# facebookresearch/habitat-lab

Hardware: AMD Instinct MI355X
Metric: env-steps/sec (SPS) PointNav RGB-D 256x256, 64 envs x 128 rollout (higher is better)
Workload: dtype f32; 1 GPU; PointNav SimpleCNN+GRU, 64 envs x 128 steps, 256x256 RGB-D synthetic; envs_per_gpu=64, rollout_steps=128, ppo_epoch=4, num_mini_batch=4, parallelism=dp1

## Files before the change

habitat-lab_amd/csrc/engine.hip:

```cpp
#include <string.h>

#include <algorithm>

#include <string>
#include <vector>

#include "engine.h"

using namespace hab;

static void plan_tm_workspace(hab_policy* e, Arena& wk);
void add_tail_params(hab_policy* e) {
    const hab_policy_desc& d = e->d;
    const int H = d.hidden;
    const std::string rn = "net.state_encoder.rnn.";
    for (int l = 0; l < d.rnn_layers; ++l) {
        const int in = l == 0 ? e->rnn_in : H;
        const std::string sfx = "_l" + std::to_string(l);
        e->i_wih.push_back(add_param(e, rn + "weight_ih" + sfx, {e->G_ * H, in}));
        e->i_whh.push_back(add_param(e, rn + "weight_hh" + sfx, {e->G_ * H, H}));
        e->i_bih.push_back(add_param(e, rn + "bias_ih" + sfx, {e->G_ * H}));
        e->i_bhh.push_back(add_param(e, rn + "bias_hh" + sfx, {e->G_ * H}));
    }
    if (d.action_dist == HAB_DIST_GAUSSIAN) {
// ... 434 lines not shown
        HAB_TRY(rnn_frag_init(hidden0 + (size_t)l * H, rows, hidden_env_stride, masks, rows, frag_env, frag_start, F, H,
                              e->WK + e->w_hinit + (size_t)l * F * H, s, env_first_frame));
        if (e->d.rnn_type == HAB_RNN_LSTM)
            HAB_TRY(rnn_frag_init(hidden0 + (size_t)(L + l) * H, rows, hidden_env_stride, masks, rows, frag_env, frag_start, F, H,
                                  e->WK + e->w_cinit + (size_t)l * F * H, s, env_first_frame));
    }
    return HAB_OK;
}
static int rnn_tm_forward(hab_policy* e, const hab_obs* obs, const int* rows, const float* hidden0, int hidden_env_stride,
                          const uint8_t* masks, int B, int n, hipStream_t stream) {
    float* W = e->WK;
    const int H = e->d.hidden, L = e->L, NC = e->form.chunks, T = B / n, Tc = (T + NC - 1) / NC;
    HAB_TRY(tm_setup(e, 2 * NC + 4));
    hipStream_t sB = e->s2;
    uint8_t* fmask = reinterpret_cast<uint8_t*>(W + e->w_fmask);
    HAB_TRY(rnn_tm_prepare(masks, rows, B, fmask, reinterpret_cast<int*>(W + e->w_iota), stream));
    HAB_TRY(rnn_state_init(e, hidden0, hidden_env_stride, rows, masks, nullptr, nullptr, n, nullptr, stream));
    for (int c = 0; c < NC; ++c) {
        const int t0 = c * Tc, t1 = std::min(T, t0 + Tc);
        if (t0 >= t1) break;
        HAB_TRY(encoder_forward(e, obs, masks, rows, B, stream, t0 * n, (t1 - t0) * n));
        HAB_TRY(tm_order(e, c, stream, sB));
        for (int l = 0; l < L; ++l) {
            Probe pr(e, HAB_PROBE_RNN_FWD, sB);
            HAB_TRY(rnn_tm_layer_forward(e->d.rnn_type, H, layer_params(e, l), layer_work(e, l), layer_x(e, l), layer_ld(e, l),
                                         W + e->w_hinit + (size_t)l * n * H, W + e->w_cinit + (size_t)l * n * H, fmask, n, T, t0, t1,
                                         W + e->w_ws2, e->ws2_floats, sB));
        }
    }
    return tm_order(e, NC, sB, stream);
}
static int rnn_packed_forward(hab_policy* e, const int* rows, const float* hidden0, int hidden_env_stride, const uint8_t* masks,
                              const hab_pack_info* pack, int n, hipStream_t stream) {
    float* W = e->WK;
    const int H = e->d.hidden, L = e->L;
    const PackInfo pk = pack_info(pack, n);
    HAB_TRY(rnn_state_init(e, hidden0, hidden_env_stride, rows, masks, pk.frag_env, pk.frag_start, pk.F, pack->env_first_frame, stream));
    if (e->form.wave) {
        RnnLayerParams lps[4]; RnnWork wks[4]; const float* hin[4]; const float* cin[4];
        for (int l = 0; l < L; ++l) {
            lps[l] = layer_params(e, l); wks[l] = layer_work(e, l);
            hin[l] = W + e->w_hinit + (size_t)l * pk.F * H; cin[l] = W + e->w_cinit + (size_t)l * pk.F * H;
        }
        Probe pr(e, HAB_PROBE_RNN_FWD, stream);
        const int rc = rnn_seq_wave_forward(e->d.rnn_type, H, L, lps, wks, layer_x(e, 0), layer_ld(e, 0), hin, cin, pk, W + e->w_ws,
                                            e->ws_floats, stream);
        return rc == 1 ? HAB_ERR_UNSUPPORTED : rc;
    }
    for (int l = 0; l < L; ++l) {
        Probe pr(e, HAB_PROBE_RNN_FWD, stream);
        HAB_TRY(rnn_seq_layer_forward(e->d.rnn_type, H, layer_params(e, l), layer_work(e, l), layer_x(e, l), layer_ld(e, l),
                                      W + e->w_hinit + (size_t)l * pk.F * H, W + e->w_cinit + (size_t)l * pk.F * H, pk, W + e->w_ws,
                                      e->ws_floats, stream));
    }
    return HAB_OK;
}

extern "C" int hab_policy_evaluate(hab_policy* e, const hab_obs* obs, const int* rows, const float* hidden0,
                                   int hidden_env_stride, const uint8_t* masks, const int64_t* actions,
                                   const hab_pack_info* pack, int B, int n, float* value, float* log_prob, float* entropy,
                                   hipStream_t stream) {
    if (!e || !e->P || !obs || !hidden0 || !masks || !actions || !pack || B <= 0 || n <= 0 || B > e->d.max_frames) return HAB_ERR_ARG;
    if (!pack->env_first_frame && (B % n)) return HAB_ERR_ARG;
    if (pack->P != B || pack->F <= 0 || pack->F > B || pack->max_len <= 0) return HAB_ERR_ARG;
    float* W = e->WK;
    const int H = e->d.hidden, L = e->L;
    e->form = rnn_form(e, rows, pack, B, n);
    if (e->form.chunks > 0) {
        HAB_TRY(rnn_tm_forward(e, obs, rows, hidden0, hidden_env_stride, masks, B, n, stream));
    } else {
        HAB_TRY(encoder_forward(e, obs, masks, rows, B, stream));
        HAB_TRY(rnn_packed_forward(e, rows, hidden0, hidden_env_stride, masks, pack, n, stream));
    }
    const float* feats = W + e->w_out[L - 1];
    if (e->d.action_dist == HAB_DIST_GAUSSIAN) {
        GaussHeadsArgs ga;
        ga.B = B; ga.H = H; ga.A = e->d.num_actions; ga.K = e->head_K; ga.flags = e->d.gauss_flags; ga.mode = 0;
        ga.min_std = e->d.gauss_min_std; ga.max_std = e->d.gauss_max_std;
        ga.feats = feats; ga.feats_ld = H; ga.w = e->p(e->i_aw); ga.b = e->p(e->i_ab);
        ga.std_param = e->i_astd >= 0 ? e->p(e->i_astd) : nullptr; ga.w_critic = e->p(e->i_cw); ga.b_critic = e->p(e->i_cb);
        ga.actions_in = reinterpret_cast<const float*>(actions); ga.rows = rows; ga.noise = nullptr; ga.actions_out = nullptr;
        ga.value = value ? value : W + e->w_value; ga.logp = log_prob ? log_prob : W + e->w_logp;
        ga.entropy = entropy ? entropy : W + e->w_ent; ga.saved = W + e->w_gsaved;
        HAB_TRY(gauss_heads_forward(ga, stream));
    } else {
    HeadsArgs ha;
        ha.B = B; ha.H = H; ha.A = e->d.num_actions; ha.mode = 0;
        ha.feats = feats; ha.feats_ld = H; ha.w_actor = e->p(e->i_aw); ha.b_actor = e->p(e->i_ab); ha.w_critic = e->p(e->i_cw); ha.b_critic = e->p(e->i_cb);
        ha.actions_in = actions; ha.rows = rows; ha.noise = nullptr; ha.actions_out = nullptr;
        ha.value = value ? value : W + e->w_value; ha.logp = log_prob ? log_prob : W + e->w_logp;
        ha.entropy = entropy ? entropy : W + e->w_ent;
        ha.probs = W + e->w_probs; ha.logits_n = W + e->w_logitsn;
        HAB_TRY(heads_forward(ha, stream));
    }
    e->last_B = B;
    e->last_n = pack->env_first_frame ? 0 : n;
    e->last_masks = masks;
    return HAB_OK;
}

extern "C" int hab_policy_final_hidden(hab_policy* e, float* hidden_out, hipStream_t stream) {
    if (!e || !hidden_out || e->last_B <= 0 || e->last_n <= 0) return HAB_ERR_ARG;
    const int H = e->d.hidden, L = e->L, n = e->last_n, B = e->last_B;
    const int Lh = e->d.rnn_type == HAB_RNN_LSTM ? 2 * L : L;
    for (int l = 0; l < L; ++l) {
        HAB_TRY(copy_rows(e->WK + e->w_out[l] + (size_t)(B - n) * H, nullptr, H, hidden_out + (size_t)l * H, Lh * H, n, H, stream));
        if (e->d.rnn_type == HAB_RNN_LSTM)
            HAB_TRY(copy_rows(e->WK + e->w_c[l] + (size_t)(B - n) * H, nullptr, H, hidden_out + (size_t)(L + l) * H, Lh * H, n, H, stream));
    }
    return HAB_OK;
}

__global__ void add_rows_kernel(float* __restrict__ dst, const float* __restrict__ src, long long n) {
    for (long long i = (long long)blockIdx.x * blockDim.x + threadIdx.x; i < n; i += (long long)gridDim.x * blockDim.x) dst[i] += src[i];
}
__global__ void add_masked_cols_kernel(float* __restrict__ dst, int ldd, const float* __restrict__ src, const float* __restrict__ x, int ldx,
                                       int B, int H) {
    const long long n = (long long)B * H;
    for (long long i = (long long)blockIdx.x * blockDim.x + threadIdx.x; i < n; i += (long long)gridDim.x * blockDim.x) {
        const int f = (int)(i / H), c = (int)(i % H);
        if (x[(size_t)f * ldx + c] > 0.f) dst[(size_t)f * ldd + c] += src[i];
    }
}
extern "C" int hab_policy_set_extra_grads(hab_policy* e, const float* d_rnn_output, const float* d_perception_embed) {
    if (!e) return HAB_ERR_ARG;
    if (d_perception_embed && e->Cin == 0) return HAB_ERR_ARG;
    e->xg_feat = d_rnn_output; e->xg_perc = d_perception_embed;
    return HAB_OK;
}

static int cnn_dgrad(hab_policy* e, int64_t f0, int nB, hipStream_t s) {
    float* W = e->WK;
    float* ws = W + e->w_ws;
    const int64_t m1 = (int64_t)e->c1.Ho() * e->c1.Wo() * 32, m2 = (int64_t)e->c2.Ho() * e->c2.Wo() * 64, m3 = e->fc_in;
    ConvDesc c2 = e->c2, c3 = e->c3;
    c2.B = c3.B = nB;
    { Probe pr(e, HAB_PROBE_FC_DGRAD, s);
      HAB_TRY(linear_dgrad(W + e->w_drnnin + f0 * e->rnn_ld, e->rnn_ld, e->PK + e->pk_fc, e->fc_in, nullptr, 0, 0, W + e->w_da3 + f0 * m3,
                           e->fc_in, nB, e->fc_in, e->d.hidden, 0, ws, e->ws_floats, s)); }
    { Probe pr(e, HAB_PROBE_CONV3_DGRAD, s);
      HAB_TRY(conv_dgrad(c3, W + e->w_da3 + f0 * m3, e->PK + e->pk_c3d, W + e->w_a2 + f0 * m2, nullptr, W + e->w_da2 + f0 * m2, ws,
                         e->ws_floats, s)); }
    { Probe pr(e, HAB_PROBE_CONV2_DGRAD, s);
      HAB_TRY(conv_dgrad(c2, W + e->w_da2 + f0 * m2, e->PK + e->pk_c2d, W + e->w_a1 + f0 * m1, nullptr, W + e->w_da1 + f0 * m1, ws,
                         e->ws_floats, s)); }
    return HAB_OK;
}
static int rnn_tm_backward(hab_policy* e, int B, hipStream_t stream) {
    float* W = e->WK;
    const int H = e->d.hidden, L = e->L, n = e->last_n, T = B / n, NC = e->form.chunks, Tc = (T + NC - 1) / NC;
    hipStream_t sB = e->s2;
    const uint8_t* fmask = reinterpret_cast<const uint8_t*>(W + e->w_fmask);
    const int* iota = reinterpret_cast<const int*>(W + e->w_iota);
    HAB_TRY(tm_order(e, NC + 1, stream, sB));
    for (int c = NC - 1; c >= 0; --c) {
        const int t0 = c * Tc, t1 = std::min(T, t0 + Tc);
        if (t0 >= t1) continue;
        for (int l = L - 1; l >= 0; --l) {
            Probe pr(e, HAB_PROBE_RNN_BWD, sB);
            HAB_TRY(rnn_tm_layer_backward(e->d.rnn_type, H, layer_params(e, l), layer_work(e, l), layer_dout(e, l), layer_dx(e, l), layer_ld(e, l),
                                          l == 0 ? layer_x(e, 0) : nullptr, layer_ld(e, l), H, fmask, iota, n, T, t0, t1,
                                          W + e->w_scratch + (size_t)l * 2 * n * H, W + e->w_ws2, e->ws2_floats, sB));
        }
        if (!e->rn) {
            HAB_TRY(tm_order(e, NC + 2 + c, sB, stream));
            HAB_TRY(cnn_dgrad(e, (int64_t)t0 * n, (t1 - t0) * n, stream));
        }
    }
    for (int l = L - 1; l >= 0; --l)
        HAB_TRY(rnn_tm_layer_param_grads(e->d.rnn_type, H, layer_params(e, l), layer_work(e, l), layer_x(e, l), layer_ld(e, l), B, W + e->w_ws2,
                                         e->ws2_floats, sB));
    return HAB_OK;
}
static int rnn_packed_backward(hab_policy* e, const hab_pack_info* pack, hipStream_t stream) {
    float* W = e->WK;
    const int H = e->d.hidden, L = e->L;
    const PackInfo pk = pack_info(pack, e->last_n);
    const bool blind0 = !e->rn && e->Cin == 0, nofc = e->Cin == 0;
    const float* x0 = layer_x(e, 0);
    if (e->form.wave) {
        RnnLayerParams lps[4]; RnnWork wks[4]; const float* wiht[4];
        for (int l = 0; l < L; ++l) { lps[l] = layer_params(e, l); wks[l] = layer_work(e, l); wiht[l] = l ? e->PK + e->pk_wiht[l] : nullptr; }
        Probe pr(e, HAB_PROBE_RNN_BWD, stream);
        const int rc = rnn_seq_wave_backward(e->d.rnn_type, H, L, lps, wiht, wks, x0, e->rnn_ld, layer_dout(e, L - 1), blind0 ? nullptr : layer_dx(e, 0),
                                             e->rnn_ld, nofc ? nullptr : x0, e->rnn_ld, nofc ? 0 : H, pk, W + e->w_scratch, W + e->w_ws, e->ws_floats,
                                             stream);
        return rc == 1 ? HAB_ERR_UNSUPPORTED : rc;
    }
    for (int l = L - 1; l >= 0; --l) {
        Probe pr(e, HAB_PROBE_RNN_BWD, stream);
        HAB_TRY(rnn_seq_layer_backward(e->d.rnn_type, H, layer_params(e, l), layer_work(e, l), layer_x(e, l), layer_ld(e, l), layer_dout(e, l),
                                       (blind0 && l == 0) ? nullptr : layer_dx(e, l), layer_ld(e, l), (l == 0 && !nofc) ? x0 : nullptr,
                                       layer_ld(e, l), nofc ? 0 : H, pk, W + e->w_scratch, W + e->w_ws, e->ws_floats, stream));
    }
    return HAB_OK;
}

static int policy_backward_impl(hab_policy* e, const hab_obs* obs, const int* rows, const int64_t* actions,
                                const hab_pack_info* pack, const float* d_value, const float* d_log_prob,
                                const float* d_entropy, hipStream_t stream) {
    if (!e || !e->P || !e->G || !obs || !actions || !pack || !d_value || !d_log_prob || !d_entropy || e->last_B <= 0)
        return HAB_ERR_ARG;
    e->comm_err = HAB_OK;
    float* W = e->WK;
    float* ws = W + e->w_ws;
    const int H = e->d.hidden, L = e->L, B = e->last_B, A = e->d.num_actions;
    e->cur_stream = stream;
    e->comm_first = -1;
    const float* feats = W + e->w_out[L - 1];
    if (e->d.action_dist == HAB_DIST_GAUSSIAN) {
        const int K = e->head_K;
        GaussHeadsBwdArgs gb;
        gb.B = B; gb.H = H; gb.A = A; gb.K = K; gb.d_value = d_value; gb.d_logp = d_log_prob; gb.d_entropy = d_entropy;
        gb.actions = reinterpret_cast<const float*>(actions); gb.rows = rows; gb.saved = W + e->w_gsaved;
        gb.w = e->p(e->i_aw); gb.w_critic = e->p(e->i_cw); gb.dfeat = W + e->w_dfeat; gb.dz = W + e->w_dzv; gb.dv_out = W + e->w_dv;
        HAB_TRY(gauss_heads_backward(gb, stream));
        HAB_TRY(linear_wgrad(W + e->w_dzv, 8, feats, H, e->g(e->i_aw), H, B, K, H, 0, 0, 0, ws, e->ws_floats, stream));
        HAB_TRY(colsum(W + e->w_dzv, 8, B, K, e->g(e->i_ab), 0, ws, e->ws_floats, stream));
        if (e->i_astd >= 0) HAB_TRY(colsum(W + e->w_dzv + A, 8, B, A, e->g(e->i_astd), 0, ws, e->ws_floats, stream));
        HAB_TRY(linear_wgrad(W + e->w_dv, 1, feats, H, e->g(e->i_cw), H, B, 1, H, 0, 0, 0, ws, e->ws_floats, stream));
        HAB_TRY(colsum(W + e->w_dv, 1, B, 1, e->g(e->i_cb), 0, ws, e->ws_floats, stream));
    } else {
    HeadsBwdArgs hb;
        hb.B = B; hb.H = H; hb.A = A; hb.d_value = d_value; hb.d_logp = d_log_prob; hb.d_entropy = d_entropy;
        hb.actions = actions; hb.rows = rows; hb.probs = W + e->w_probs; hb.logits_n = W + e->w_logitsn;
        hb.w_actor = e->p(e->i_aw); hb.w_critic = e->p(e->i_cw); hb.dfeat = W + e->w_dfeat; hb.dzv = W + e->w_dzv; hb.dv_out = W + e->w_dv;
        HAB_TRY(heads_backward(hb, stream));
        HAB_TRY(linear_wgrad(W + e->w_dzv, 8, feats, H, e->g(e->i_aw), H, B, A, H, 0, 0, 0, ws, e->ws_floats, stream));
        HAB_TRY(linear_wgrad(W + e->w_dv, 1, feats, H, e->g(e->i_cw), H, B, 1, H, 0, 0, 0, ws, e->ws_floats, stream));
        HAB_TRY(colsum(W + e->w_dzv, 8, B, A, e->g(e->i_ab), 0, ws, e->ws_floats, stream));
        HAB_TRY(colsum(W + e->w_dv, 1, B, 1, e->g(e->i_cb), 0, ws, e->ws_floats, stream));
    }
    const int NC = e->form.chunks;
    if (e->xg_feat || e->xg_perc) {
        if (NC > 0) return HAB_ERR_UNSUPPORTED;
        if (e->xg_feat) {
            add_rows_kernel<<<(int)std::min<long long>(1024, cdivl((long long)B * H, 256)), 256, 0, stream>>>(W + e->w_dfeat, e->xg_feat, (long long)B * H);
            HAB_LAUNCH_CHECK();
        }
    }
    if (NC > 0) {
        HAB_TRY(rnn_tm_backward(e, B, stream));
    } else {
        HAB_TRY(rnn_packed_backward(e, pack, stream));
        if (e->xg_perc) {
            add_masked_cols_kernel<<<(int)std::min<long long>(1024, cdivl((long long)B * H, 256)), 256, 0, stream>>>(
                W + e->w_drnnin, e->rnn_ld, e->xg_perc, W + e->w_rnnin, e->rnn_ld, B, H);
            HAB_LAUNCH_CHECK();
        }
        if (!e->rn && e->Cin == 0) {
            grad_tail_ready(e, e->i_wih[0]);
            return HAB_OK;
        }
    }
    if (e->rn) {
        if (NC > 0) HAB_TRY(tm_order(e, 2 * NC + 3, e->s2, stream));
        Probe pr(e, HAB_PROBE_ENC_BWD, stream);
        return resnet_encoder_backward(e, obs, e->last_masks, rows, B, stream);
    }
    const float* dfc = W + e->w_drnnin;
    { Probe pr(e, HAB_PROBE_FC_WGRAD, stream);
      HAB_TRY(linear_wgrad(dfc, e->rnn_ld, W + e->w_a3, e->fc_in, e->g(e->i_fcw), e->fc_in, B, H, e->fc_in, 32, e->fc_in / 32, 0,
                           ws, e->ws_floats, stream)); }
    HAB_TRY(colsum(dfc, e->rnn_ld, B, H, e->g(e->i_fcb), 0, ws, e->ws_floats, stream));
    if (NC > 0) HAB_TRY(tm_order(e, 2 * NC + 3, e->s2, stream));
    grad_tail_ready(e, e->i_fcw);
    if (NC == 0) HAB_TRY(cnn_dgrad(e, 0, B, stream));
    ConvDesc c1 = e->c1, c2 = e->c2, c3 = e->c3;
    c1.B = c2.B = c3.B = B;
    { Probe pr(e, HAB_PROBE_CONV3_WGRAD, stream);
      HAB_TRY(conv_wgrad(c3, W + e->w_a2, W + e->w_da3, e->g(e->i_c3w), e->g(e->i_c3b), ws, e->ws_floats, stream)); }
    { Probe pr(e, HAB_PROBE_CONV2_WGRAD, stream);
      HAB_TRY(conv_wgrad(c2, W + e->w_a1, W + e->w_da2, e->g(e->i_c2w), e->g(e->i_c2b), ws, e->ws_floats, stream)); }
    ObsView ov;
    ov.rgb = e->d.has_rgb ? obs->rgb : nullptr; ov.depth = e->d.has_depth ? obs->depth : nullptr; ov.rows = rows;
    ov.H = e->d.H; ov.W = e->d.W; ov.C = e->Cin;
    { Probe pr(e, HAB_PROBE_CONV1_WGRAD, stream);
      HAB_TRY(obs_conv_wgrad(c1, ov, W + e->w_da1, e->g(e->i_c1w), e->g(e->i_c1b), ws, e->ws_floats, stream)); }
    return HAB_OK;
}
extern "C" int hab_policy_backward(hab_policy* e, const hab_obs* obs, const int* rows, const int64_t* actions,
                                   const hab_pack_info* pack, const float* d_value, const float* d_log_prob,
                                   const float* d_entropy, hipStream_t stream) {
    const int rc = policy_backward_impl(e, obs, rows, actions, pack, d_value, d_log_prob, d_entropy, stream);
    if (e) e->xg_feat = e->xg_perc = nullptr;
    return (rc == HAB_OK && e && e->comm_err != HAB_OK) ? e->comm_err : rc;
}

extern "C" int hab_policy_tap(hab_policy* e, int which, const float** ptr, int64_t* floats) {
    if (!e || !ptr || !floats || e->last_B <= 0) return HAB_ERR_ARG;
    const int64_t B = e->last_B;
    float* W = e->WK;
    if (e->rn && which != HAB_TAP_RNN_IN && which != HAB_TAP_RNN_OUT) return resnet_tap(e, which, ptr, floats);
    if (!e->rn && e->Cin == 0 && (which == HAB_TAP_CONV1 || which == HAB_TAP_CONV2 || which == HAB_TAP_CONV3)) return HAB_ERR_ARG;
    switch (which) {
        case HAB_TAP_CONV1: *ptr = W + e->w_a1; *floats = B * e->c1.Ho() * e->c1.Wo() * 32; break;
        case HAB_TAP_CONV2: *ptr = W + e->w_a2; *floats = B * e->c2.Ho() * e->c2.Wo() * 64; break;
        case HAB_TAP_CONV3: *ptr = W + e->w_a3; *floats = B * e->fc_in; break;
        case HAB_TAP_RNN_IN: *ptr = W + e->w_rnnin; *floats = B * e->rnn_ld; break;
        case HAB_TAP_RNN_OUT: *ptr = W + e->w_out[e->L - 1]; *floats = B * e->d.hidden; break;
        default: return HAB_ERR_ARG;
    }
    return HAB_OK;
}
```

habitat-lab_amd/csrc/gemm_ops.hip:

```cpp
#include "igemm.h"
#include "igemm_dma.h"
#include "igemm_dma_wgrad.h"
#include "igemm_bf3.h"
#include "igemm_bf3_ws.h"
#include "dense_bf3.h"
#include "obs_conv_bf3.h"
#include "obs_conv_bf3_ws.h"
#include "obs_conv_patch.h"
#include "wgrad3x3_bf3.h"
#include "conv2_fwd_strip.h"
#include "conv2_dgrad_strip.h"
#include "obs_wgrad_bf3.h"
#include "conv_patch_bf3.h"
#include "wgrad3x3_patch.h"
#include "prob_build.h"
#include <stdlib.h>

#include <atomic>

#include "../../include/habitat_amd.h"

namespace hab {

static bool no_dma() { static const bool v = hab_env_flag("HAB_NO_DMA"); return v; }
static bool no_merged_dgrad() { static const bool v = hab_env_flag("HAB_NO_MERGED_DGRAD"); return v; }
static bool no_patch() { static const bool v = hab_env_flag("HAB_NO_PATCH"); return v; }
static std::atomic<int> g_bf3_mode{-1};
static int bf3_mode() {
    int m = g_bf3_mode.load(std::memory_order_relaxed);
    if (m < 0) {
        static const int from_env = hab_env_int("HAB_BF3", 2047);
        int expected = -1;
        g_bf3_mode.compare_exchange_strong(expected, from_env, std::memory_order_relaxed);
        m = g_bf3_mode.load(std::memory_order_relaxed);
    }
    return m;
}
int matrix_path_bits() { return bf3_mode(); }
extern "C" int hab_set_matrix_path(int mode) {
    const int prev = bf3_mode();
    if (mode >= 0) g_bf3_mode.store(mode, std::memory_order_relaxed);
    return prev;
}


template <class P, int TM, int TN, int WM, int WN>
static int bf3_launch(const P& p, float* ws, size_t ws_floats, int target_blocks, hipStream_t stream) {
    constexpr bool WS_SHAPE = P::A_RC && P::B_RC && TM == 2 && TN == 2 && WM == 2 && WN == 2;
    if constexpr (WS_SHAPE) {
        constexpr int ws_min_k = 2048;
        if ((bf3_mode() & 32) && p.K >= ws_min_k) return igemm_bf3_ws_launch<P, TM, TN, WM, WN, 4>(p, ws, ws_floats, target_blocks, stream);
    }
    return igemm_bf3_launch<P, TM, TN, WM, WN>(p, ws, ws_floats, target_blocks, stream);
}

template <class P>
static int run_igemm(const P& p, float* ws, size_t ws_floats, hipStream_t stream, int target_blocks = 1024) {
    if (P::A_RC || P::B_RC) target_blocks = 256;
    constexpr bool WG = !P::A_RC && !P::B_RC && AKv<P>::value == 4;
    if constexpr (P::A_RC && P::B_RC) {
        if ((bf3_mode() & 1) && p.M > 64) {
            if (p.N <= 32) return bf3_launch<P, 2, 1, 4, 1>(p, ws, ws_floats, target_blocks, stream);
            if (p.N <= 64) {
                if (p.M >= 256 * 512 && p.K >= 576) return bf3_launch<P, 2, 2, 4, 1>(p, ws, ws_floats, target_blocks, stream);
                return bf3_launch<P, 1, 2, 4, 1>(p, ws, ws_floats, target_blocks, stream);
            }
            return bf3_launch<P, 2, 2, 2, 2>(p, ws, ws_floats, target_blocks, stream);
        }
    } else if constexpr (AKv<P>::value == 4) {
        if ((bf3_mode() & 4) && p.M > 64) {
            if (p.N <= 32) {
                if constexpr (WG) {
                    if (p.M % 96 == 0 || cdiv(p.M, 96) * 96 < cdiv(p.M, 256) * 256)
                        return bf3_launch<P, 1, 1, 3, 1>(p, ws, ws_floats, target_blocks, stream);
                }
                return bf3_launch<P, 2, 1, 4, 1>(p, ws, ws_floats, target_blocks, stream);
            }
            if (p.N <= 64) {
                if constexpr (WG) {
                    if (p.M % 96 == 0 || cdiv(p.M, 96) * 96 < cdiv(p.M, 128) * 128)
                        return bf3_launch<P, 1, 2, 3, 1>(p, ws, ws_floats, target_blocks, stream);
                }
                return bf3_launch<P, 1, 2, 4, 1>(p, ws, ws_floats, target_blocks, stream);
            }
            return bf3_launch<P, 2, 2, 2, 2>(p, ws, ws_floats, target_blocks, stream);
        }
    }
    if constexpr (std::is_same_v<P, ConvFwdProb> || std::is_same_v<P, ConvDgradProb>) {
        if (p.dma_ok() && p.M > 64 && !no_dma()) {
            if (p.N <= 32) return igemm_dma_launch<P, 2, 1, 4, 1, false>(p, ws, ws_floats, target_blocks, stream);
            if (p.N <= 64) return igemm_dma_launch<P, 1, 2, 4, 1, false>(p, ws, ws_floats, target_blocks, stream);
            if (p.N <= 128) return igemm_dma_launch<P, 2, 2, 2, 2, true>(p, ws, ws_floats, target_blocks, stream);
        }
    }
    if (p.N <= 32) {
        if (p.M <= 64) return igemm_launch<P, 1, 1, 2, 1>(p, ws, ws_floats, target_blocks, stream);
        if constexpr (WG) {
            if (p.M % 96 == 0 || cdiv(p.M, 96) * 96 < cdiv(p.M, 256) * 256)
                return igemm_launch<P, 1, 1, 3, 1>(p, ws, ws_floats, target_blocks, stream);
        }
        return igemm_launch<P, 2, 1, 4, 1>(p, ws, ws_floats, target_blocks, stream);
    } else if (p.N <= 64) {
        if (p.M <= 64) return igemm_launch<P, 1, 1, 2, 2>(p, ws, ws_floats, target_blocks, stream);
        if constexpr (WG) {
            if (p.M % 96 == 0 || cdiv(p.M, 96) * 96 < cdiv(p.M, 128) * 128)
                return igemm_launch<P, 1, 2, 3, 1>(p, ws, ws_floats, target_blocks, stream);
        }
        return igemm_launch<P, 1, 2, 4, 1>(p, ws, ws_floats, target_blocks, stream);
    } else {
        if (p.M <= 64) return igemm_launch<P, 1, 2, 2, 2>(p, ws, ws_floats, target_blocks, stream);
        return igemm_launch<P, 2, 2, 2, 2>(p, ws, ws_floats, target_blocks, stream);
    }
}

int conv_fwd(const ConvDesc& d, const float* x, const float* wf, const float* bias, float* y, int relu, float* ws,
             size_t ws_floats, hipStream_t stream) {
    ConvFwdProb p;
    HAB_TRY(build(p, d, x, wf, bias, y, relu));
    if ((bf3_mode() & 256) && (bf3_mode() & 1)) {
        const int rc = conv2_fwd_strip(p, ws, ws_floats, stream);
        if (rc != 1) return rc;
    }
    if ((bf3_mode() & 16) && d.stride == 1 && d.KH == 3 && d.KW == 3 && p.M > 64) {
        PatchGeom gq{};
        gq.in = x; gq.Hi = d.H; gq.Wi = d.W; gq.Ci = d.C; gq.Ho = p.g.Ho; gq.Wo = p.g.Wo; gq.KH = 3; gq.KW = 3;
        gq.off_h = -d.pad; gq.off_w = -d.pad; gq.flip = 0;
        const int rc = conv_patch_bf3_dispatch(p, gq, ws, ws_floats, stream);
        if (rc != 1) return rc;
    }
    return run_igemm(p, ws, ws_floats, stream);
}
int64_t obs_conv_weight_image_floats() { return ((int64_t)OCP_W_ELEMS + 1) / 2 + 4; }
int obs_conv_weight_image(const float* wf, int Cout, int KH, int KW, int C, void* img, hipStream_t stream) {
    return obs_conv_patch_weight_image(wf, Cout, KH, KW, C, reinterpret_cast<unsigned short*>(img), stream);
}
int obs_conv_fwd(const ConvDesc& d, const ObsView& obs, const float* wf, const float* bias, float* y, int relu, float* ws,
                 size_t ws_floats, hipStream_t stream, const void* wimg) {
    ObsConvFwdProb p;
    HAB_TRY(build(p, d, obs, wf, bias, y, relu));
    if ((bf3_mode() & 64) && (bf3_mode() & 2) && p.quad) {
        const int rc = obs_conv_patch_launch(p, ws, ws_floats, stream, reinterpret_cast<const unsigned short*>(wimg));
        if (rc != 1) return rc;
    }
    if ((bf3_mode() & 32) && (bf3_mode() & 2) && p.quad && p.M > 64) {
        const int rc = obs_conv_bf3_ws_launch(p, ws, ws_floats, stream);
        if (rc != 1) return rc;
    }
    if ((bf3_mode() & 2) && p.quad && p.M > 64) {
        const int rc = obs_conv_bf3_launch<2>(p, ws, ws_floats, stream);
        if (rc != 1) return rc;
    }
    return run_igemm(p, ws, ws_floats, stream);
}
__global__ void dgrad_empty_class_kernel(ConvDgradProb p) {
    const long long total = (long long)p.g.B * p.Hc * p.Wc * p.N;
    for (long long e = (long long)blockIdx.x * blockDim.x + threadIdx.x; e < total; e += (long long)gridDim.x * blockDim.x)
        p.store((int)(e / p.N), (int)(e % p.N), 0.f);
}

int conv_dgrad(const ConvDesc& d, const float* dy, const float* wd, const float* mask, const float* add, float* dx,
               float* ws, size_t ws_floats, hipStream_t stream) {
    if ((bf3_mode() & 512) && (bf3_mode() & 1)) {
        const int rc = conv2_dgrad_strip(d, dy, wd, mask, add, dx, stream);
        if (rc != 1) return rc;
    }
    if (d.stride > 1 && !no_dma() && !no_merged_dgrad()) {
        ConvDgradMergedProb q;
        HAB_TRY(check_conv(d));
        q.g = make_geom(d);
        if (ConvDgradMergedProb::applicable(q.g)) {
            q.dy = dy; q.w = wd; q.mask = mask; q.add = add; q.dx = dx;
            q.finish();
            if ((bf3_mode() & 1) && q.M > 64) {
                if (q.N <= 32) return bf3_launch<ConvDgradMergedProb, 2, 1, 4, 1>(q, ws, ws_floats, 256, stream);
                if (q.N <= 64) return bf3_launch<ConvDgradMergedProb, 1, 2, 4, 1>(q, ws, ws_floats, 256, stream);
                return bf3_launch<ConvDgradMergedProb, 2, 2, 2, 2>(q, ws, ws_floats, 256, stream);
            }
            if (q.dma_ok()) {
                if (q.N <= 32) return igemm_dma_launch<ConvDgradMergedProb, 2, 1, 4, 1, false>(q, ws, ws_floats, 1024, stream);
                if (q.N <= 64) return igemm_dma_launch<ConvDgradMergedProb, 1, 2, 4, 1, false>(q, ws, ws_floats, 1024, stream);
                return igemm_dma_launch<ConvDgradMergedProb, 2, 2, 2, 2, false>(q, ws, ws_floats, 1024, stream);
            }
        }
    }
    for (int ph = 0; ph < d.stride; ++ph)
        for (int pw = 0; pw < d.stride; ++pw) {
            ConvDgradProb p;
            HAB_TRY(build(p, d, dy, wd, mask, add, dx, ph, pw));
            if (p.Hc <= 0 || p.Wc <= 0) continue;
            if ((bf3_mode() & 16) && d.stride == 1 && d.KH == 3 && d.KW == 3 && p.M > 64 && p.K > 0) {
                PatchGeom gq{};
                gq.in = dy; gq.Hi = p.g.Ho; gq.Wi = p.g.Wo; gq.Ci = d.Cout; gq.Ho = d.H; gq.Wo = d.W; gq.KH = 3; gq.KW = 3;
                gq.off_h = d.pad - 2; gq.off_w = d.pad - 2; gq.flip = 1;
                const int rc = conv_patch_bf3_dispatch(p, gq, ws, ws_floats, stream);
                if (rc == HAB_OK) continue;
                if (rc != 1) return rc;
            }
            if (p.K <= 0) {
                p.M = d.B * p.Hc * p.Wc;
                dgrad_empty_class_kernel<<<1024, 256, 0, stream>>>(p);
                HAB_LAUNCH_CHECK();
                continue;
            }
            HAB_TRY(run_igemm(p, ws, ws_floats, stream));
        }
    return HAB_OK;
}
int conv_wgrad(const ConvDesc& d, const float* x, const float* dy, float* dw_oihw, float* dbias, float* ws, size_t ws_floats,
               hipStream_t stream) {
    ConvWgradProb p;
    HAB_TRY(build(p, d, x, dy, dw_oihw, dbias));
    if (ws && (bf3_mode() & 8) && (bf3_mode() & 128) && wgrad3x3_bf3_shape(p)) {
        const int rc = wgrad3x3_bf3(p, ws, ws_floats, stream);
        if (rc != 1) return rc;
    }
    if (ws && wgrad3x3_patch_ok(p) && !no_patch() && !(bf3_mode() & 8)) {
        ConvWgradProb q = p;
        q.colsum = nullptr;
        if (dbias) HAB_TRY(colsum(dy, p.N, p.K, p.N, dbias, 0, ws, ws_floats, stream));
        return wgrad3x3_patch(q, ws, ws_floats, stream);
    }
    if (ws && d.pad == 0 && p.N <= 32 && !no_dma() && !(bf3_mode() & 8)) {
        ConvWgradProb q = p;
        q.colsum = nullptr;
        if (wgrad_dma_ok(q)) {
            if (dbias) HAB_TRY(colsum(dy, p.N, p.K, p.N, dbias, 0, ws, ws_floats, stream));
            if ((q.M % 288 == 0) || (cdiv(q.M, 288) * 288 < cdiv(q.M, 256) * 256)) return igemm_dma_wgrad_launch<3, 3, 1>(q, ws, ws_floats, 1024, stream);
            return igemm_dma_wgrad_launch<2, 4, 1>(q, ws, ws_floats, 1024, stream);
        }
    }
    return run_igemm(p, ws, ws_floats, stream);
}
int obs_conv_wgrad(const ConvDesc& d, const ObsView& obs, const float* dy, float* dw_oihw, float* dbias, float* ws,
                   size_t ws_floats, hipStream_t stream) {
    ObsConvWgradProb p;
    HAB_TRY(build(p, d, obs, dy, dw_oihw, dbias));
    if ((bf3_mode() & 2) && p.quad && p.K > 4096) {
        const int rc = obs_wgrad_bf3_launch(p, ws, ws_floats, stream);
        if (rc != 1) return rc;
    }
    return run_igemm(p, ws, ws_floats, stream);
}
static bool dense_on() { return (bf3_mode() & 1024) && (bf3_mode() & 1); }
static bool dense_worth(long long M, long long N, long long K) {
    if (bf3_mode() & 2048) return true;
    static const long long min_flop = (long long)hab_env_int("HAB_DENSE_MIN_MFLOP", 4000) * 1000000LL;
    return 2 * M * N * K >= min_flop;
}
int linear_fwd(const float* x, int ldx, const float* w, int ldw, const float* bias, float* y, int ldy, int M, int N, int K,
               int relu, int accumulate, float* ws, size_t ws_floats, hipStream_t stream) {
    LinearFwdProb p;
    HAB_TRY(build(p, x, ldx, w, ldw, bias, y, ldy, M, N, K, relu, accumulate));
    if (dense_on() && dense_worth(M, N, K)) {
        DenseArgs g{};
        g.M = M; g.N = N; g.K = K; g.a = x; g.lda = ldx; g.b = w; g.ldb = ldw; g.c = y; g.ldc = ldy; g.bias = bias; g.relu = relu;
        g.accumulate = accumulate; g.partial = ws;
        g.a_bytes = ((long long)(M - 1) * ldx + K) * 4; g.b_bytes = ((long long)(N - 1) * ldw + K) * 4;
        if (dense_bf3_ok(g, false, false)) {
            g.nsplit = ws ? dense_bf3_splits(g, ws_floats) : 1;
            HAB_TRY((dense_bf3_launch<0, 0>(g, stream)));
            if (g.nsplit > 1) {
                igemm_splitk_reduce<LinearFwdProb>(p, ws, g.nsplit, stream);
                HAB_LAUNCH_CHECK();
            }
            return HAB_OK;
        }
    }
    return run_igemm(p, ws, ws_floats, stream);
}
int linear_dgrad(const float* dy, int lddy, const float* w, int ldw, const float* mask, int ldmask, int mask_cols, float* dx,
                 int lddx, int M, int Nin, int Kout, int accumulate, float* ws, size_t ws_floats, hipStream_t stream) {
    LinearDgradProb p;
    HAB_TRY(build(p, dy, lddy, w, ldw, mask, ldmask, mask_cols, dx, lddx, M, Nin, Kout, accumulate));
    if (dense_on() && !mask && dense_worth(M, Nin, Kout)) {
        DenseArgs g{};
        g.M = M; g.N = Nin; g.K = Kout; g.a = dy; g.lda = lddy; g.b = w; g.ldb = ldw; g.c = dx; g.ldc = lddx; g.accumulate = accumulate;
        g.partial = ws;
        g.a_bytes = ((long long)(M - 1) * lddy + Kout) * 4; g.b_bytes = ((long long)(Kout - 1) * ldw + Nin) * 4;
        if (dense_bf3_ok(g, false, true)) {
            g.nsplit = ws ? dense_bf3_splits(g, ws_floats) : 1;
            HAB_TRY((dense_bf3_launch<0, 1>(g, stream)));
            if (g.nsplit > 1) {
                igemm_splitk_reduce<LinearDgradProb>(p, ws, g.nsplit, stream);
                HAB_LAUNCH_CHECK();
            }
            return HAB_OK;
        }
    }
    return run_igemm(p, ws, ws_floats, stream);
}
int linear_wgrad(const float* dy, int lddy, const float* x, int ldx, float* dw, int lddw, int Mrows, int Nout, int Kin,
                 int perm_c, int perm_hw, int accumulate, float* ws, size_t ws_floats, hipStream_t stream) {
    LinearWgradProb p;
    HAB_TRY(build(p, dy, lddy, x, ldx, dw, lddw, Mrows, Nout, Kin, perm_c, perm_hw, accumulate));
    if (dense_on() && dense_worth(Nout, Kin, Mrows)) {
        DenseArgs g{};
        g.M = Nout; g.N = Kin; g.K = Mrows; g.a = dy; g.lda = lddy; g.b = x; g.ldb = ldx; g.c = dw; g.ldc = lddw; g.accumulate = accumulate;
        g.perm_c = perm_c; g.perm_hw = perm_hw; g.partial = ws;
        g.a_bytes = ((long long)(Mrows - 1) * lddy + Nout) * 4; g.b_bytes = ((long long)(Mrows - 1) * ldx + Kin) * 4;
        if (dense_bf3_ok(g, true, true)) {
            g.nsplit = ws ? dense_bf3_splits(g, ws_floats) : 1;
            HAB_TRY((dense_bf3_launch<1, 1>(g, stream)));
            if (g.nsplit > 1) {
                igemm_splitk_reduce<LinearWgradProb>(p, ws, g.nsplit, stream);
                HAB_LAUNCH_CHECK();
            }
            return HAB_OK;
        }
    }
    return run_igemm(p, ws, ws_floats, stream);
}

__global__ void __launch_bounds__(256) colsum_stage1(const float* __restrict__ a, int lda, int M, int N, int rows_per_block,
                                                     float* __restrict__ partial) {
    const int cw = N < 64 ? N : 64;
    const int rl = 256 / cw;
    const int c = threadIdx.x % cw, r = threadIdx.x / cw;
    const int n = blockIdx.x * cw + c;
    __shared__ float sm[256];
    const int m_begin = blockIdx.y * rows_per_block, m_end = min(M, m_begin + rows_per_block);
    float s0 = 0.f, s1 = 0.f;
    if (r < rl && n < N) {
        int m = m_begin + r;
        for (; m + rl < m_end; m += 2 * rl) {
            s0 += a[(size_t)m * lda + n];
            s1 += a[(size_t)(m + rl) * lda + n];
        }
        if (m < m_end) s0 += a[(size_t)m * lda + n];
    }
    sm[threadIdx.x] = s0 + s1;
    __syncthreads();
    if (r == 0 && n < N) {
        float t = 0.f;
        for (int q = 0; q < rl; ++q) t += sm[q * cw + c];
        partial[(size_t)blockIdx.y * N + n] = t;
    }
}
__global__ void __launch_bounds__(256) colsum_stage2(const float* __restrict__ partial, int nblocks, int N, float* __restrict__ out,
                                                     int accumulate) {
    __shared__ float sm[4][64];
    const int c = threadIdx.x & 63, r = threadIdx.x >> 6;
    const int n = blockIdx.x * 64 + c;
    float s0 = 0.f, s1 = 0.f, s2 = 0.f, s3 = 0.f;
    if (n < N) {
        int b = r;
        for (; b + 12 < nblocks; b += 16) {
            s0 += partial[(size_t)b * N + n];
            s1 += partial[(size_t)(b + 4) * N + n];
            s2 += partial[(size_t)(b + 8) * N + n];
            s3 += partial[(size_t)(b + 12) * N + n];
        }
        for (; b < nblocks; b += 4) s0 += partial[(size_t)b * N + n];
    }
    const float s = (s0 + s1) + (s2 + s3);
    sm[r][c] = s;
    __syncthreads();
    if (r == 0 && n < N) {
        const float t = (sm[0][c] + sm[1][c]) + (sm[2][c] + sm[3][c]);
        out[n] = accumulate ? out[n] + t : t;
    }
}

int colsum(const float* a, int lda, int M, int N, float* out, int accumulate, float* ws, size_t ws_floats, hipStream_t stream) {
    if (M <= 0 || N <= 0 || !a || !out || !ws) return HAB_ERR_ARG;
    const int cw = N < 64 ? N : 64;
    const int colblocks = cdiv(N, cw);
    int chunks = cdiv(1024, colblocks);
    if (chunks > cdiv(M, 16)) chunks = cdiv(M, 16);
    while (chunks > 1 && (size_t)chunks * N > ws_floats) chunks >>= 1;
    if ((size_t)chunks * N > ws_floats) return HAB_ERR_ARG;
    const int rpb = cdiv(M, chunks);
    chunks = cdiv(M, rpb);
    colsum_stage1<<<dim3(colblocks, chunks), 256, 0, stream>>>(a, lda, M, N, rpb, ws);
    HAB_LAUNCH_CHECK();
    colsum_stage2<<<cdiv(N, 64), 256, 0, stream>>>(ws, chunks, N, out, accumulate);
    HAB_LAUNCH_CHECK();
    return HAB_OK;
}

__global__ void repack_conv_kernel(const float* __restrict__ w, float* __restrict__ wf, float* __restrict__ wd, int Cout,
                                   int Cin, int KH, int KW, int cpad) {
    const int total = Cout * cpad * KH * KW;
    for (int e = blockIdx.x * blockDim.x + threadIdx.x; e < total; e += gridDim.x * blockDim.x) {
        const int ci = e % cpad;
        int t = e / cpad;
        const int kw = t % KW; t /= KW;
        const int kh = t % KH;
        const int co = t / KH;
        const float v = (ci < Cin) ? w[(((size_t)co * Cin + ci) * KH + kh) * KW + kw] : 0.f;
// ... 145 lines not shown
```

Before: 61740 env-steps/s.

## Add patch-based obs conv1 wgrad kernel and start RNN backward earlier

Adds a new MFMA bf16x3 weight-gradient kernel for the 8x8 stride-4 first conv on raw RGB-D observations. It stages row-band patches in an LDS ring so overlapping input rows are reused across output rows, and it is enabled by default through a new mode bit. It also moves the stream-ordering event for the RNN backward stream to right after the heads backward, so RNN backward can overlap the head weight-gradient GEMMs. The new kernel adds more bf16 split arithmetic and a split-K reduction. It only covers a narrow shape set and falls back otherwise.

Measured after the change: 54950 env-steps/s. -11.0%, worse.

```diff
diff --git a/habitat-lab_amd/csrc/engine.hip b/habitat-lab_amd/csrc/engine.hip
--- a/habitat-lab_amd/csrc/engine.hip
+++ b/habitat-lab_amd/csrc/engine.hip
@@ -610,7 +610,6 @@
     hipStream_t sB = e->s2;
     const uint8_t* fmask = reinterpret_cast<const uint8_t*>(W + e->w_fmask);
     const int* iota = reinterpret_cast<const int*>(W + e->w_iota);
-    HAB_TRY(tm_order(e, NC + 1, stream, sB));
     for (int c = NC - 1; c >= 0; --c) {
         const int t0 = c * Tc, t1 = std::min(T, t0 + Tc);
         if (t0 >= t1) continue;
@@ -666,6 +665,7 @@
     e->cur_stream = stream;
     e->comm_first = -1;
     const float* feats = W + e->w_out[L - 1];
+    const int NC = e->form.chunks;
     if (e->d.action_dist == HAB_DIST_GAUSSIAN) {
         const int K = e->head_K;
         GaussHeadsBwdArgs gb;
@@ -673,6 +673,7 @@
         gb.actions = reinterpret_cast<const float*>(actions); gb.rows = rows; gb.saved = W + e->w_gsaved;
         gb.w = e->p(e->i_aw); gb.w_critic = e->p(e->i_cw); gb.dfeat = W + e->w_dfeat; gb.dz = W + e->w_dzv; gb.dv_out = W + e->w_dv;
         HAB_TRY(gauss_heads_backward(gb, stream));
+        if (NC > 0) HAB_TRY(tm_order(e, NC + 1, stream, e->s2));
         HAB_TRY(linear_wgrad(W + e->w_dzv, 8, feats, H, e->g(e->i_aw), H, B, K, H, 0, 0, 0, ws, e->ws_floats, stream));
         HAB_TRY(colsum(W + e->w_dzv, 8, B, K, e->g(e->i_ab), 0, ws, e->ws_floats, stream));
         if (e->i_astd >= 0) HAB_TRY(colsum(W + e->w_dzv + A, 8, B, A, e->g(e->i_astd), 0, ws, e->ws_floats, stream));
@@ -684,12 +685,12 @@
         hb.actions = actions; hb.rows = rows; hb.probs = W + e->w_probs; hb.logits_n = W + e->w_logitsn;
         hb.w_actor = e->p(e->i_aw); hb.w_critic = e->p(e->i_cw); hb.dfeat = W + e->w_dfeat; hb.dzv = W + e->w_dzv; hb.dv_out = W + e->w_dv;
         HAB_TRY(heads_backward(hb, stream));
+        if (NC > 0) HAB_TRY(tm_order(e, NC + 1, stream, e->s2));
         HAB_TRY(linear_wgrad(W + e->w_dzv, 8, feats, H, e->g(e->i_aw), H, B, A, H, 0, 0, 0, ws, e->ws_floats, stream));
         HAB_TRY(linear_wgrad(W + e->w_dv, 1, feats, H, e->g(e->i_cw), H, B, 1, H, 0, 0, 0, ws, e->ws_floats, stream));
         HAB_TRY(colsum(W + e->w_dzv, 8, B, A, e->g(e->i_ab), 0, ws, e->ws_floats, stream));
         HAB_TRY(colsum(W + e->w_dv, 1, B, 1, e->g(e->i_cb), 0, ws, e->ws_floats, stream));
     }
-    const int NC = e->form.chunks;
     if (e->xg_feat || e->xg_perc) {
         if (NC > 0) return HAB_ERR_UNSUPPORTED;
         if (e->xg_feat) {
diff --git a/habitat-lab_amd/csrc/gemm_ops.hip b/habitat-lab_amd/csrc/gemm_ops.hip
--- a/habitat-lab_amd/csrc/gemm_ops.hip
+++ b/habitat-lab_amd/csrc/gemm_ops.hip
@@ -11,6 +11,7 @@
 #include "conv2_fwd_strip.h"
 #include "conv2_dgrad_strip.h"
 #include "obs_wgrad_bf3.h"
+#include "obs_wgrad_patch.h"
 #include "conv_patch_bf3.h"
 #include "wgrad3x3_patch.h"
 #include "prob_build.h"
@@ -29,7 +30,7 @@
 static int bf3_mode() {
     int m = g_bf3_mode.load(std::memory_order_relaxed);
     if (m < 0) {
-        static const int from_env = hab_env_int("HAB_BF3", 2047);
+        static const int from_env = hab_env_int("HAB_BF3", 2047 | 8192);
         int expected = -1;
         g_bf3_mode.compare_exchange_strong(expected, from_env, std::memory_order_relaxed);
         m = g_bf3_mode.load(std::memory_order_relaxed);
@@ -235,6 +236,10 @@
                    size_t ws_floats, hipStream_t stream) {
     ObsConvWgradProb p;
     HAB_TRY(build(p, d, obs, dy, dw_oihw, dbias));
+    if ((bf3_mode() & 2) && (bf3_mode() & 8192) && p.quad && p.K > 1024) {
+        const int rc = obs_wgrad_patch_launch(p, ws, ws_floats, stream);
+        if (rc != 1) return rc;
+    }
     if ((bf3_mode() & 2) && p.quad && p.K > 4096) {
         const int rc = obs_wgrad_bf3_launch(p, ws, ws_floats, stream);
         if (rc != 1) return rc;
diff --git a/habitat-lab_amd/csrc/obs_wgrad_patch.h b/habitat-lab_amd/csrc/obs_wgrad_patch.h
--- /dev/null
+++ b/habitat-lab_amd/csrc/obs_wgrad_patch.h
@@ -0,0 +1,229 @@
+#pragma once
+#include "obs_wgrad_bf3.h"
+
+namespace hab {
+
+constexpr int OWP_P = 72;
+constexpr int OWP_SLOT = 24 * OWP_P + 32;
+constexpr int OWP_RING = 8 * OWP_SLOT;
+constexpr int OWP_BP = 32 * OWP_P;
+constexpr size_t OWP_LDS_BYTES = (size_t)(OWP_RING + 2 * 3 * OWP_BP) * 2;
+static_assert(OWP_LDS_BYTES >= 256 * 32 * 4, "the cross-wave reduction reuses the tile buffers");
+static_assert(OWP_LDS_BYTES % 16 == 0 && (OWP_SLOT * 2) % 16 == 0, "16-byte fragment reads");
+
+struct ObsWgradPatchGeom {
+    FastDiv dHo;
+    int tiles, tiles_per_wg;
+};
+
+__global__ void __launch_bounds__(256, 2) obs_wgrad_patch_kernel(const ObsConvWgradProb p, const ObsWgradPatchGeom gg, float* __restrict__ partial) {
+    extern __shared__ __attribute__((aligned(16))) unsigned short smem16[];
+    unsigned short* T = smem16;
+    unsigned short* B0 = T + OWP_RING;
+    unsigned short* B1 = B0 + 3 * OWP_BP;
+
+    const int t = threadIdx.x;
+    const int lane = t & 63, wave = t >> 6;
+    const int li = lane & 31, hi = lane >> 5;
+    const ConvGeom& g = p.g;
+
+    const int qpr = g.W >> 2;
+    const int a_r = t / qpr, a_x4 = t - a_r * qpr;
+    const bool a_ok = t < g.W;
+    const size_t a_pix = (size_t)(a_ok ? a_r : 0) * g.W + 4 * (a_ok ? a_x4 : 0);
+    const int b_coq = t >> 5, b_kr = t & 31;
+    const bool b_col_ok = b_coq * 4 < p.N;
+
+    const int tile_begin = blockIdx.x * gg.tiles_per_wg;
+    const int tile_end = min(gg.tiles, tile_begin + gg.tiles_per_wg);
+
+    for (int i = t; i < (int)(OWP_LDS_BYTES / 16); i += 256) reinterpret_cast<u32x4*>(smem16)[i] = u32x4{0u, 0u, 0u, 0u};
+    __syncthreads();
+
+    struct Rgb12 { uint32_t d0, d1, d2; };
+    Rgb12 rg_new, rg_old;
+    f32x4 dp_new, dp_old, b_raw[2];
+    rg_old.d0 = rg_old.d1 = rg_old.d2 = 0; dp_old = zero4();
+    f32x4 cs = zero4();
+    const bool has_cs = p.colsum != nullptr;
+
+    auto fetch = [&](int tile) {
+        int img, ho;
+        gg.dHo.divmod(tile, img, ho);
+        const size_t frame = (size_t)p.obs.srow(img) * g.H;
+        const size_t pix = (frame + 4 * ho + 4) * g.W + a_pix;
+        rg_new = *reinterpret_cast<const Rgb12*>(p.obs.rgb + pix * 3);
+        dp_new = ld4(p.obs.depth + pix);
+        if (ho == 0 || tile == tile_begin) {
+            const size_t pix0 = pix - (size_t)4 * g.W;
+            rg_old = *reinterpret_cast<const Rgb12*>(p.obs.rgb + pix0 * 3);
+            dp_old = ld4(p.obs.depth + pix0);
+        }
+        const float* dyrow = p.dy + ((size_t)tile * g.Wo) * p.N + b_coq * 4;
+#pragma unroll
+        for (int r = 0; r < 2; ++r) {
+            const bool ok = b_col_ok & (b_kr * 2 + r < g.Wo);
+            b_raw[r] = ok ? ld4(dyrow + (size_t)(b_kr * 2 + r) * p.N) : zero4();
+        }
+    };
+    auto put_group = [&](const Rgb12& rg, const f32x4& dp, int half) {
+        unsigned short* dst = T + (half * 4 + a_r) * OWP_SLOT + a_x4;
+        const unsigned d[3] = {rg.d0, rg.d1, rg.d2};
+#pragma unroll
+        for (int e = 0; e < 12; ++e)
+            dst[e * OWP_P] = (unsigned short)(__float_as_uint((float)((d[e >> 2] >> (8 * (e & 3))) & 0xffu)) >> 16);
+        unsigned w[2][3];
+        bf3_split2(dp[0], dp[1], w[0][0], w[0][1], w[0][2]);
+        bf3_split2(dp[2], dp[3], w[1][0], w[1][1], w[1][2]);
+#pragma unroll
+        for (int pl = 0; pl < 3; ++pl)
+#pragma unroll
+            for (int f = 0; f < 4; ++f)
+                dst[(12 + pl * 4 + f) * OWP_P] = (unsigned short)((f & 1) ? (w[f >> 1][pl] >> 16) : w[f >> 1][pl]);
+    };
+    auto stage = [&](int tile) {
+        int img, ho;
+        gg.dHo.divmod(tile, img, ho);
+        if (a_ok) {
+            if (ho == 0 || tile == tile_begin) put_group(rg_old, dp_old, ho & 1);
+            put_group(rg_new, dp_new, (ho + 1) & 1);
+        }
+        if (has_cs) cs += b_raw[0] + b_raw[1];
+#pragma unroll
+        for (int e = 0; e < 4; ++e) {
+            unsigned w[3];
+            bf3_split2(b_raw[0][e], b_raw[1][e], w[0], w[1], w[2]);
+            const int off = (b_coq * 4 + e) * OWP_P + b_kr * 2;
+#pragma unroll
+            for (int pl = 0; pl < 3; ++pl) {
+                *reinterpret_cast<unsigned*>(B0 + pl * OWP_BP + off) = w[pl];
+                B1[pl * OWP_BP + off + 1] = (unsigned short)w[pl];
+                B1[pl * OWP_BP + off + 2] = (unsigned short)(w[pl] >> 16);
+            }
+        }
+    };
+
+    const int koff = wave * 16 + hi * 8;
+    int a_off[4], a_odd[4];
+#pragma unroll
+    for (int j = 0; j < 3; ++j) {
+        const int rr = 32 * j + li, kh = rr / 12;
+        a_off[j] = kh * OWP_SLOT + (rr - kh * 12) * OWP_P + koff;
+        a_odd[j] = kh < 4 ? 4 * OWP_SLOT : -4 * OWP_SLOT;
+    }
+    a_off[3] = (li >> 2) * OWP_SLOT + (12 + (li & 3)) * OWP_P + koff;
+    a_odd[3] = li < 16 ? 4 * OWP_SLOT : -4 * OWP_SLOT;
+
+    f32x16 acc[8];
+#pragma unroll
+    for (int i = 0; i < 8; ++i)
+#pragma unroll
+        for (int v = 0; v < 16; ++v) acc[i][v] = 0.0f;
+
+    const unsigned sf = wave >= 2 ? 0x80008000u : 0u;
+    u32x4 sign_flip;
+    sign_flip[0] = sf; sign_flip[1] = sf; sign_flip[2] = sf; sign_flip[3] = sf;
+    if (tile_begin < tile_end) fetch(tile_begin);
+    for (int tile = tile_begin; tile < tile_end; ++tile) {
+        stage(tile);
+        __syncthreads();
+        if (tile + 1 < tile_end) fetch(tile + 1);
+        int img, ho;
+        gg.dHo.divmod(tile, img, ho);
+        const bool par = ho & 1;
+        bf16x8 b[2][3];
+#pragma unroll
+        for (int sh = 0; sh < 2; ++sh)
+#pragma unroll
+            for (int pl = 0; pl < 3; ++pl) {
+                u32x4 raw = *reinterpret_cast<const u32x4*>((sh ? B1 : B0) + pl * OWP_BP + li * OWP_P + koff);
+                raw ^= sign_flip;
+                b[sh][pl] = __builtin_bit_cast(bf16x8, raw);
+            }
+#pragma unroll
+        for (int j = 0; j < 3; ++j) {
+            const bf16x8 a = *reinterpret_cast<const bf16x8*>(T + a_off[j] + (par ? a_odd[j] : 0));
+#pragma unroll
+            for (int sh = 0; sh < 2; ++sh)
+#pragma unroll
+                for (int pl = 2; pl >= 0; --pl) acc[sh * 3 + j] = __builtin_amdgcn_mfma_f32_32x32x16_bf16(a, b[sh][pl], acc[sh * 3 + j], 0, 0, 0);
+        }
+        {
+            const unsigned short* src = T + a_off[3] + (par ? a_odd[3] : 0);
+            bf16x8 a[3];
+#pragma unroll
+            for (int pl = 0; pl < 3; ++pl) a[pl] = *reinterpret_cast<const bf16x8*>(src + pl * 4 * OWP_P);
+            constexpr int PA[6] = {2, 0, 1, 1, 0, 0}, PB[6] = {0, 2, 1, 0, 1, 0};
+#pragma unroll
+            for (int sh = 0; sh < 2; ++sh)
+#pragma unroll
+                for (int q = 0; q < 6; ++q) acc[6 + sh] = __builtin_amdgcn_mfma_f32_32x32x16_bf16(a[PA[q]], b[sh][PB[q]], acc[6 + sh], 0, 0, 0);
+        }
+        __syncthreads();
+    }
+
+    float* red = reinterpret_cast<float*>(smem16);
+    for (int w = 0; w < 4; ++w) {
+        if (wave == w) {
+#pragma unroll
+            for (int mt = 0; mt < 8; ++mt)
+#pragma unroll
+                for (int v = 0; v < 16; ++v) {
+                    const int rrow = mt * 32 + (v & 3) + 8 * (v >> 2) + 4 * hi;
+                    float* dst = red + rrow * 32 + li;
+                    *dst = (w == 0 ? 0.f : *dst) + (w >= 2 ? -acc[mt][v] : acc[mt][v]);
+                }
+        }
+        __syncthreads();
+    }
+    const int MP = p.M + (has_cs ? 1 : 0);
+    float* slab = partial + (size_t)blockIdx.x * MP * p.N;
+    for (int e = t; e < 256 * 32; e += 256) {
+        const int rrow = e >> 5, co = e & 31;
+        int i;
+        if (rrow < 192) {
+            const int sh = rrow >= 96, rr = rrow - 96 * sh, kh = rr / 12, fc = rr - kh * 12, f = fc / 3;
+            i = (kh * 8 + sh * 4 + f) * 4 + (fc - 3 * f);
+        } else {
+            const int d = rrow - 192;
+            i = ((d & 31) >> 2) * 32 + (d >> 5) * 16 + (d & 3) * 4 + 3;
+        }
+        if (co < p.N) slab[(size_t)i * p.N + co] = red[e];
+    }
+    if (has_cs) {
+        __syncthreads();
+        *reinterpret_cast<f32x4*>(red + t * 4) = cs;
+        __syncthreads();
+        if (t < p.N) {
+            float s = 0.f;
+            for (int q = 0; q < 32; ++q) s += red[((t >> 2) * 32 + q) * 4 + (t & 3)];
+            slab[(size_t)p.M * p.N + t] = s;
+        }
+    }
+}
+
+inline int obs_wgrad_patch_launch(const ObsConvWgradProb& p, float* ws, size_t ws_floats, hipStream_t stream) {
+    const ConvGeom& g = p.g;
+    if (!p.quad || g.KH != 8 || g.KW != 8 || g.stride != 4 || g.pad != 0 || p.M != 256 || p.N > 32 || p.N < 4 || (p.N & 3) || (g.W & 3) || g.W > 256 ||
+        g.W < 8 || g.H < 8 || g.Ho < 1 || g.Wo != (g.W >> 2) - 1 || g.B < 1 || !ws)
+        return 1;
+    ObsWgradPatchGeom gg;
+    gg.tiles = g.B * g.Ho;
+    gg.dHo = FastDiv(g.Ho);
+    constexpr int wgs_env = 512;
+    int wgs = gg.tiles < wgs_env ? gg.tiles : wgs_env;
+    const int MP = p.M + (p.colsum ? 1 : 0);
+    while (wgs > 1 && (size_t)wgs * MP * p.N > ws_floats) wgs >>= 1;
+    if ((size_t)wgs * MP * p.N > ws_floats) return 1;
+    gg.tiles_per_wg = cdiv(gg.tiles, wgs);
+    wgs = cdiv(gg.tiles, gg.tiles_per_wg);
+    static const hipError_t attr_err = hipFuncSetAttribute(reinterpret_cast<const void*>(obs_wgrad_patch_kernel), hipFuncAttributeMaxDynamicSharedMemorySize, (int)OWP_LDS_BYTES);
+    if (attr_err != hipSuccess) return (int)attr_err;
+    obs_wgrad_patch_kernel<<<wgs, 256, OWP_LDS_BYTES, stream>>>(p, gg, ws);
+    HAB_LAUNCH_CHECK();
+    igemm_splitk_reduce<ObsConvWgradProb>(p, ws, wgs, stream);
+    HAB_LAUNCH_CHECK();
+    return HAB_OK;
+}
+
+}
```
